# Francis-Fan-create/SCaSML_GP

Measured on AMD Instinct MI355X. Metric: Euler-Maruyama path-steps/sec + L2 rel-error, Grad_Dependent_Nonlinear d=100 n=3, higher is better.
Workload: dtype f32

## Files before the change

scasml_gp_amd/csrc/gp_eval_compat_mfma.hip:

```cpp
#include <stdlib.h>
#include <type_traits>

#include "gp_common.hpp"
#include "gp_mfma16.hpp"

namespace scasml {

constexpr int kHutch = 5;

typedef _Float16 h16x2 __attribute__((ext_vector_type(2)));
typedef float f32x2 __attribute__((ext_vector_type(2)));

struct CompatIdxF {
    int32_t i[kHutch];
};

struct GpCompatArgs {
    const float *points;
    const float *model;
    int32_t idx[kHutch];
    float4 *out4;
    float *lap;
    int64_t n_inf;
    int32_t n_pad, kp, d, first_bdy_tile;
    float a, sigma, mu;
    int32_t eq_id;
    int32_t round_out;
    const uint8_t *site_kinds;
    int64_t rows_per_site;
    const int32_t *site_order;
    int32_t n_listed;
};

template <bool R16>
struct Pair {
    using T = std::conditional_t<R16, h16x2, f32x2>;
    T v;
    __device__ __forceinline__ Pair(float a, float b) {
        if constexpr (R16) v = __builtin_convertvector((f32x2){a, b}, h16x2);
        else v = (f32x2){a, b};
    }
    __device__ __forceinline__ float lo() const { return (float)v.x; }
    __device__ __forceinline__ float hi() const { return (float)v.y; }
};

__device__ __forceinline__ float pin(float x) {
    asm("" : "+v"(x));
    return x;
}

template <int KS, int PLANES>
__device__ __forceinline__ void compat_mfma_lam(const float4 *lds_a, const s16x8 (&xb)[PLANES][KS], f32x16 &acc, int lane, float acc0) {
#pragma unroll
    for (int r = 0; r < 16; ++r) acc[r] = acc0;
    constexpr int NA = PLANES == 2 ? 1 : 2;
    Frag a[NA];
    if constexpr (NA == 2) a[0].f = lds_a[lane];
#pragma unroll
    for (int s = 0; s < KS; ++s) {
        const int cur = NA == 2 ? (s & 1) : 0, nxt = cur ^ 1;
        if constexpr (NA == 2) {
            if (s + 1 < KS) a[nxt].f = lds_a[(s + 1) * 64 + lane];
        } else {
            a[0].f = lds_a[s * 64 + lane];
        }
        Frag b0;
        b0.v = xb[0][s];
        if constexpr (PLANES == 2) {
            Frag b1;
            b1.v = xb[1][s];
            acc = __builtin_amdgcn_mfma_f32_32x32x16_f16(a[cur].h, b1.h, acc, 0, 0, 0);
        }
        acc = __builtin_amdgcn_mfma_f32_32x32x16_f16(a[cur].h, b0.h, acc, 0, 0, 0);
        __builtin_amdgcn_sched_barrier(0);
    }
}

struct CompatPoint {
    float sx, tx, ax0, sx2, wxa, wxb;
};
struct CompatConsts {
    float a, ad, c4, c10;
};

template <int GEOM, int FORM, bool BDY, bool R16>
__device__ __forceinline__ void compat_epilogue(const float *rows_lds, const f32x16 &lam, const f32x16 &G, int half, const CompatPoint &p,
                                                const CompatConsts &c, float &au, float &at, float &ad, float &al) {
    const float4 *cb = reinterpret_cast<const float4 *>(__builtin_assume_aligned(rows_lds + 4 * 8 * half, 16));
    constexpr int NQ = (BDY || GEOM == 1) ? 1 : 2;
    float4 q[1][NQ];
    auto fetch = [&](int r, float4 (&dst)[NQ]) {
        const int row = (r & 3) + 8 * (r >> 2);
#pragma unroll
        for (int i = 0; i < NQ; ++i) dst[i] = cb[row * 2 + i];
    };
#pragma unroll
    for (int r = 0; r < 16; ++r) {
        const int cur = 0;
        fetch(r, q[0]);
        __builtin_amdgcn_sched_barrier(0);
        const float kap = pin(__builtin_amdgcn_exp2f(lam[r]));
        if constexpr (GEOM == 0) {
            const float vsy = q[cur][0].x, vty = q[cur][0].y, c0 = q[cur][0].z;
            if constexpr (BDY && FORM == 1) {
                const Pair<R16> k0(kap, 0.0f);
                au = fmaf(c0, k0.lo(), au);
            } else {
                const float pp = p.tx - vty, ss = p.sx - vsy;
                const float e1 = pin(pp * kap), e2 = pin(ss * kap);
                if constexpr (BDY) {
                    const Pair<R16> k01(kap, e1), k2(e2, 0.0f);
                    au = fmaf(c0, k01.lo(), au);
                    if constexpr (FORM == 0) at = fmaf(-c0, k01.hi(), at);
                    if constexpr (FORM != 1) ad = fmaf(-c0, k2.lo(), ad);
                } else {
                    const float cL = q[cur][0].w, ct = q[cur][1].x, cS = q[cur][1].y;
                    if constexpr (FORM == 1) {
                        const Pair<R16> k01(kap, e1), k2(e2, 0.0f);
                        au = fmaf(cS, k2.lo(), fmaf(ct, k01.hi(), fmaf(c0, k01.lo(), au)));
                    } else {
                        const float e4 = pin(pp * e2);
                        const float e5 = pin(fmaf(-ss, e2, c.ad * kap));
                        if constexpr (FORM == 2) {
                            const Pair<R16> k01(kap, e1), k24(e2, e4), k5(e5, 0.0f);
                            au = fmaf(cS, k24.lo(), fmaf(ct, k01.hi(), fmaf(c0, k01.lo(), au)));
                            ad = fmaf(cS, k5.lo(), fmaf(-ct, k24.hi(), fmaf(-c0, k24.lo(), ad)));
                        } else {
                            const float e3 = fmaf(-pp, e1, c.a * kap);
                            const float g0 = G[r];
                            const float e6 = fmaf(g0, g0 - c.c4, -c.c10) * kap;
                            const Pair<R16> k01(kap, e1), k23(e2, e3), k45(e4, e5), k6(e6, 0.0f);
                            au = fmaf(cS, k23.lo(), fmaf(ct, k01.hi(), fmaf(c0, k01.lo(), au)));
                            at = fmaf(-cS, k45.lo(), fmaf(ct, k23.hi(), fmaf(-c0, k01.hi(), at)));
                            ad = fmaf(cS, k45.hi(), fmaf(-ct, k45.lo(), fmaf(-c0, k23.lo(), ad)));
                            al = fmaf(cL, k6.lo(), al);
                        }
                    }
                }
            }
        } else if constexpr (GEOM == 1) {
            const float vsy1 = q[cur][0].x, vay0 = q[cur][0].y, vwy1 = q[cur][0].z, cL = q[cur][0].w;
            const float g1 = G[r];
            const float f1 = pin(g1 * kap);
            if constexpr (FORM == 1) {
                const Pair<R16> k1(f1, 0.0f);
                au = fmaf(cL, k1.lo(), au);
            } else {
                const float m = fmaf(-(p.sx - vsy1), g1, p.wxb - vwy1);
                const float f3 = pin(m * kap);
                if constexpr (FORM == 2) {
                    const Pair<R16> k13(f1, f3);
                    au = fmaf(cL, k13.lo(), au);
                    ad = fmaf(cL, k13.hi(), ad);
                } else {
                    const float f2 = (p.tx - vay0) * f1;
                    const Pair<R16> k12(f1, f2), k3(f3, 0.0f);
                    au = fmaf(cL, k12.lo(), au);
                    at = fmaf(-cL, k12.hi(), at);
                    ad = fmaf(cL, k3.lo(), ad);
                }
            }
        } else {
            const float vsy = q[cur][0].x, vty = q[cur][0].y, vwy2 = q[cur][0].z, c0 = q[cur][0].w;
            const float g2 = G[r];
            const float h1 = g2 * kap;
            if constexpr (BDY) {
                const Pair<R16> k1(h1, 0.0f);
                al = fmaf(c0, k1.lo(), al);
            } else {
                const float ct = q[cur][1].x, cS = q[cur][1].y;
                const float h2 = (p.ax0 - vty) * h1;
                const float m = fmaf(-(p.sx2 - vsy), g2, p.wxa - vwy2);
                const float h3 = m * kap;
                const Pair<R16> k12(h1, h2), k3(h3, 0.0f);
                al = fmaf(-cS, k3.lo(), fmaf(ct, k12.hi(), fmaf(c0, k12.lo(), al)));
            }
        }
    }
}

template <int GEOM, int FORM, bool BDY>
__device__ __forceinline__ void compat_epilogue_fact(const float *rows_lds, const f32x16 &lam, const f32x16 &G, int half, const CompatPoint &p,
                                                     const CompatConsts &c, float &au, float &at, float &ad, float &al) {
    const float4 *cb = reinterpret_cast<const float4 *>(__builtin_assume_aligned(rows_lds + 4 * 8 * half, 16));
    constexpr int Q0 = GEOM == 2 ? 1 : 0;
    constexpr int NQ = (GEOM == 0 && !BDY) ? 2 : 1;
    float4 q[2][NQ];
    auto fetch = [&](int r, float4 (&dst)[NQ]) {
        const int row = (r & 3) + 8 * (r >> 2);
#pragma unroll
        for (int i = 0; i < NQ; ++i) dst[i] = cb[row * 2 + Q0 + i];
    };
    fetch(0, q[0]);
#pragma unroll
    for (int r = 0; r < 16; ++r) {
        const int cur = r & 1, nxt = cur ^ 1;
        if (r + 1 < 16) fetch(r + 1, q[nxt]);
        #ifndef SCASML_FACT_NOSCHED
        __builtin_amdgcn_sched_barrier(0);
#endif
        const float kap = __builtin_amdgcn_exp2f(lam[r]);
        if constexpr (GEOM == 0) {
            const float vsy = q[cur][0].x, vty = q[cur][0].y, c0 = q[cur][0].z;
            if constexpr (BDY) {
                const float F = c0 * kap;
                au += F;
                if constexpr (FORM == 0) at = fmaf(-(p.tx - vty), F, at);
                if constexpr (FORM != 1) ad = fmaf(-(p.sx - vsy), F, ad);
            } else {
                const float cL = q[cur][0].w, ct = q[cur][1].x, cS = q[cur][1].y;
                const float pp = p.tx - vty, ss = p.sx - vsy;
                const float E = fmaf(ct, pp, fmaf(cS, ss, c0));
                au = fmaf(kap, E, au);
                if constexpr (FORM != 1) ad = fmaf(kap, fmaf(-ss, E, q[cur][1].w), ad);
                if constexpr (FORM == 0) {
                    at = fmaf(kap, fmaf(-pp, E, q[cur][1].z), at);
                    const float g0 = G[r];
                    al = fmaf(cL * kap, fmaf(g0, g0 - c.c4, -c.c10), al);
                }
            }
        } else if constexpr (GEOM == 1) {
            const float vsy1 = q[cur][0].x, vay0 = q[cur][0].y, vwy1 = q[cur][0].z, cL = q[cur][0].w;
            const float v = cL * kap;
            if constexpr (FORM == 1) {
                au = fmaf(v, G[r], au);
            } else {
                const float w = v * G[r];
                au += w;
                ad = fmaf(-(p.sx - vsy1), w, fmaf(v, p.wxb - vwy1, ad));
                if constexpr (FORM == 0) at = fmaf(-(p.tx - vay0), w, at);
            }
        } else {
            const float ct = q[cur][0].x, cS = q[cur][0].y, e0 = q[cur][0].z, cSw = q[cur][0].w;
            if constexpr (BDY) {
                al = fmaf(kap * G[r], e0, al);
            } else {
                const float E2 = fmaf(ct, p.ax0, fmaf(cS, p.sx2, e0));
                const float t = fmaf(cS, p.wxa, -cSw);
                al = fmaf(kap, fmaf(G[r], E2, -t), al);
            }
        }
    }
}

constexpr int kStageTail = 256 + 256;

template <int KS, int BPC, bool R16, int PLANES>
__global__ __launch_bounds__(256, BPC) void gp_eval_compat_mfma_kernel(const GpCompatArgs g) {
    static_assert(PLANES == 2 || !R16, "the as-coded form keeps both point planes");
#ifndef SCASML_COMPAT_NSLOT
#define SCASML_COMPAT_NSLOT 3
#endif
    constexpr int WPB = 4, NSLOT = SCASML_COMPAT_NSLOT, AHEAD = 2;
    constexpr int STAGE = KS * 256 + kStageTail;
    constexpr int NCHUNK = STAGE / 256;
    constexpr int CLO = NCHUNK / WPB, CREM = NCHUNK % WPB;
    extern __shared__ __attribute__((aligned(16))) float lds[];
    const int lane = threadIdx.x & 63, wv = threadIdx.x >> 6;
    const int col = lane & 31, half = lane >> 5;
    const int64_t blk = blockIdx.x;
    int64_t p0 = (blk * WPB + wv) * 32;
    const int n_tiles = g.n_pad / 32;
    const int nb0 = g.first_bdy_tile < n_tiles ? g.first_bdy_tile : n_tiles;

    int form_listed = -1;
    if (g.site_order) {
        const int64_t wps = g.rows_per_site >> 5;
        bool all_u = true, all_ud = true;
        for (int w = 0; w < WPB; ++w) {
            const int64_t vs = (blk * WPB + w) / wps;
            if (vs >= g.n_listed) continue;
            const int k = g.site_kinds ? g.site_kinds[g.site_order[vs]] : 0;
            if (!(k == 1 || k == 3)) all_u = false;
            if (!(k == 1 || k == 3 || k == 4)) all_ud = false;
        }
        form_listed = all_u ? 1 : (all_ud ? 2 : 0);
        const int64_t vw = blk * WPB + wv, vs = vw / wps;
        p0 = vs < g.n_listed ? (int64_t)g.site_order[vs] * g.rows_per_site + (vw - vs * wps) * 32 : g.n_inf;
    }

    if (!g.site_order && g.site_kinds && g.rows_per_site >= 32) {
        const int64_t b0 = blk * WPB * 32;
        if (b0 < g.n_inf) {
            const int64_t b1 = (b0 + WPB * 32 < g.n_inf ? b0 + WPB * 32 : g.n_inf) - 1;
            bool unowned = true;
            for (int64_t s = b0 / g.rows_per_site; s <= b1 / g.rows_per_site; ++s)
                if (g.site_kinds[s] != 2) unowned = false;
            if (unowned) return;
        }
    }
    int form = 0;
    if (g.site_order) {
        form = form_listed;
    } else if (g.site_kinds && g.rows_per_site >= 32) {
        const int64_t b0 = blk * WPB * 32;
        const int64_t b1 = (b0 + WPB * 32 < g.n_inf ? b0 + WPB * 32 : g.n_inf) - 1;
        if (b0 < g.n_inf) {
            bool all_u = true, all_ud = true;
            for (int64_t s = b0 / g.rows_per_site; s <= b1 / g.rows_per_site; ++s) {
                const int k = g.site_kinds[s];
                if (k == 2) continue;
                if (!(k == 1 || k == 3)) all_u = false;
                if (!(k == 1 || k == 3 || k == 4)) all_ud = false;
            }
            form = all_u ? 1 : (all_ud ? 2 : 0);
        }
    }
    form = __builtin_amdgcn_readfirstlane(form);
    const int GD = form == 0 ? 3 : 2, GB = form == 0 ? 2 : 1;
    const int n_stages = nb0 * GD + (n_tiles - nb0) * GB;

    const int wvs = __builtin_amdgcn_readfirstlane(wv);
    const bool extra = wvs < CREM;
    const uint32_t lds_base = __builtin_amdgcn_readfirstlane((uint32_t)(uintptr_t)lds);
    auto stage_src = [&](int s) -> const float * {
        int tile, geom;
        if (s < nb0 * GD) {
            tile = s / GD;
            geom = s - tile * GD;
        } else {
            const int t = s - nb0 * GD;
            tile = nb0 + t / GB;
            geom = form == 0 ? 2 * (t - (t / GB) * GB) : 0;
        }
        return g.model + ((int64_t)tile * 3 + geom) * STAGE;
    };
    auto stage = [&](int s) {
        const uint32_t dst = lds_base + (uint32_t)((s % NSLOT) * STAGE) * 4u;
        const float *src = stage_src(s);
        auto chunk = [&](int c) { glds16_asm(src + c * 256, (uint32_t)lane * 16u, dst + (uint32_t)c * 1024u); };
#pragma unroll
        for (int i = 0; i < CLO; ++i) chunk(wvs + i * WPB);
        if (CREM && extra) chunk(wvs + CLO * WPB);
    };
    auto rendezvous = [&](bool newest_may_fly) {
        if (newest_may_fly) {
            if (CREM && extra) {
                asm volatile("s_waitcnt vmcnt(%0)" ::"n"(CLO + 1) : "memory");
            } else {
                asm volatile("s_waitcnt vmcnt(%0)" ::"n"(CLO) : "memory");
            }
        } else {
            asm volatile("s_waitcnt vmcnt(0)" ::: "memory");
        }
        __builtin_amdgcn_s_barrier();
        asm volatile("" ::: "memory");
    };
    stage(0);
    if (n_stages > 1) stage(1);

    const float qs = 0.5f * 1.44269504088896341f / g.a, k1 = -qs;
    const float hh = (float)g.d / (float)kHutch;
    const float ha2 = hh * g.a * g.a;
    s16x8 xb[PLANES][KS];
    float acc0 = 0.0f;
    CompatPoint pt;
    Frag qa[1], qb[1];
    {
        int64_t row = p0 + col;
        if (row >= g.n_inf) row = g.n_inf - 1;
        const float *prow = g.points + row * g.kp;
        const int kbase = half * (8 * KS);
        const float4 *src = reinterpret_cast<const float4 *>(prow + kbase);
        float pn = 0.0f, ps = 0.0f;
        const float ptime = prow[g.d], px0 = prow[0];
        const float fold = 2.0f * g.a * g.a * qs;
        auto make_planes = [&](const float (&t)[8], Frag &fh, Frag &fl) {
#pragma unroll
            for (int c = 0; c < 4; ++c) {
                const float h0 = (float)(_Float16)t[2 * c], h1 = (float)(_Float16)t[2 * c + 1];
                fh.u[c] = pack_h2(t[2 * c], t[2 * c + 1]);
                fl.u[c] = pack_h2(t[2 * c] - h0, t[2 * c + 1] - h1);
            }
        };
        float tlast[8];
#pragma unroll
        for (int s = 0; s < KS; ++s) {
            const float4 q0 = src[2 * s], q1 = src[2 * s + 1];
            const float e[8] = {q0.x, q0.y, q0.z, q0.w, q1.x, q1.y, q1.z, q1.w};
            float t[8];
#pragma unroll
            for (int c2 = 0; c2 < 8; ++c2) {
                pn = fmaf(e[c2], e[c2], pn);
                ps += e[c2];
                t[c2] = fold * e[c2];
            }
            if (s == KS - 1) {
#pragma unroll
                for (int c2 = 0; c2 < 8; ++c2) tlast[c2] = t[c2];
            } else {
                Frag fh, fl;
                make_planes(t, fh, fl);
                xb[0][s] = fh.v;
                if constexpr (PLANES == 2) xb[1][s] = fl.v;
            }
        }
        pn += __shfl_xor(pn, 32);
        ps += __shfl_xor(ps, 32);
        tlast[5] = half ? 1.0f : tlast[5];
        tlast[6] = half ? 1.0f : tlast[6];
        tlast[7] = half ? k1 * g.a * g.a * pn : tlast[7];
        {
            Frag fh, fl;
            make_planes(tlast, fh, fl);
            xb[0][KS - 1] = fh.v;
            if constexpr (PLANES == 2) xb[1][KS - 1] = fl.v;
            else acc0 = k1 * g.a * g.a * pn - (float)(_Float16)(k1 * g.a * g.a * pn);
        }
        pt.sx = g.a * (ps - ptime);
        pt.tx = g.a * ptime;
        pt.ax0 = g.a * px0;
        pt.sx2 = pt.sx - pt.ax0 + pt.tx;
        float ua[kHutch], ub[kHutch], sa = 0.0f, sb = 0.0f, na = 0.0f, nb = 0.0f;
#pragma unroll
        for (int j = 0; j < kHutch; ++j) {
            const float va = prow[g.idx[j] + 1], vb = prow[g.idx[j]];
            sa += va;
            sb += vb;
            na = fmaf(va, va, na);
            nb = fmaf(vb, vb, nb);
            ua[j] = -2.0f * ha2 * va;
            ub[j] = -2.0f * ha2 * vb;
        }
        pt.wxa = 2.0f * ha2 * sa;
        pt.wxb = 2.0f * ha2 * sb;
        auto qfrag = [&](const float (&u)[kHutch], float px, Frag &f) {
            auto hi = [](float v) { return (float)(_Float16)v; };
            if (half == 0) {
                f.u[0] = pack_h2(u[0], u[1]);
                f.u[1] = pack_h2(u[2], u[3]);
                f.u[2] = pack_h2(u[4], px);
                f.u[3] = pack_h2(px - hi(px), 1.0f);
            } else {
                f.u[0] = pack_h2(u[0] - hi(u[0]), u[1] - hi(u[1]));
                f.u[1] = pack_h2(u[2] - hi(u[2]), u[3] - hi(u[3]));
                f.u[2] = pack_h2(u[4] - hi(u[4]), 1.0f);
                f.u[3] = 0u;
            }
        };
        const float c5ah = (float)kHutch * g.a * hh;
        qfrag(ua, fmaf(ha2, na, -c5ah), qa[0]);
        qfrag(ub, fmaf(ha2, nb, -c5ah), qb[0]);
    }
    CompatConsts cc;
    cc.a = g.a;
    cc.ad = g.a * (float)g.d;
    cc.c4 = 4.0f * g.a * hh;
    cc.c10 = 10.0f * g.a * g.a * hh * hh;
    float au = 0.0f, at = 0.0f, ad = 0.0f, al = 0.0f;
    f32x16 acc, accG;
    uint32_t region;
    asm volatile("s_mov_b32 %0, -1" : "=s"(region));

    int s_now = 0;
    auto step = [&](auto geom_c, auto form_c, auto bdy_c) {
        constexpr int GEOM = decltype(geom_c)::value, FORM = decltype(form_c)::value;
        constexpr bool BDY = decltype(bdy_c)::value;
        constexpr bool NEEDG = GEOM != 0 || (FORM == 0 && !BDY);
        const int slot = s_now % NSLOT;
        if (s_now + AHEAD < n_stages) stage(s_now + AHEAD);
        const float *base = lds + slot * STAGE;
        if (region & 1) {
            compat_mfma_lam<KS, PLANES>(reinterpret_cast<const float4 *>(base), xb, acc, lane, acc0);
            if constexpr (NEEDG) {
                Frag aq;
                aq.f = reinterpret_cast<const float4 *>(base + KS * 256)[lane];
#pragma unroll
                for (int r = 0; r < 16; ++r) accG[r] = 0.0f;
                accG = __builtin_amdgcn_mfma_f32_32x32x16_f16(aq.h, GEOM == 1 ? qb[0].h : qa[0].h, accG, 0, 0, 0);
            }
        }
        if (region & 2) {
            if constexpr (R16) compat_epilogue<GEOM, FORM, BDY, true>(base + (KS + 1) * 256, acc, accG, half, pt, cc, au, at, ad, al);
            else compat_epilogue_fact<GEOM, FORM, BDY>(base + (KS + 1) * 256, acc, accG, half, pt, cc, au, at, ad, al);
        }
        rendezvous(s_now + AHEAD < n_stages);
        ++s_now;
    };
    using I0 = std::integral_constant<int, 0>;
    using I1 = std::integral_constant<int, 1>;
    using I2 = std::integral_constant<int, 2>;
    auto sweep = [&](auto form_c) {
        constexpr int FORM = decltype(form_c)::value;
        for (int jt = 0; jt < nb0; ++jt) {
            step(I0{}, form_c, std::false_type{});
            step(I1{}, form_c, std::false_type{});
            if constexpr (FORM == 0) step(I2{}, form_c, std::false_type{});
        }
        for (int jt = nb0; jt < n_tiles; ++jt) {
            step(I0{}, form_c, std::true_type{});
            if constexpr (FORM == 0) step(I2{}, form_c, std::true_type{});
        }
    };
    rendezvous(n_stages > 1);
    if (form == 2) sweep(I2{});
    else if (form == 1) sweep(I1{});
    else sweep(I0{});

    float u = au + __shfl_xor(au, 32);
    const float dt = at + __shfl_xor(at, 32);
    const float dv = ad + __shfl_xor(ad, 32);
    const float lp = al + __shfl_xor(al, 32);
    const int64_t row = p0 + col;
    if (half == 0 && row < g.n_inf) {
        if (g.round_out) u = (float)(_Float16)u;
        float eps = dt + g.mu * dv + 0.5f * g.sigma * g.sigma * lp + eq_f<float>(g.eq_id, u, g.sigma * dv, g.sigma, (float)g.d);
        if (g.round_out) eps = (float)(_Float16)eps;
        g.out4[row] = make_float4(u, dv, eps, dt);
        if (g.lap) g.lap[row] = lp;
    }
}

__global__ void gp_compat_pack_mfma_kernel(int d, float a, const float *x_dom, int n_dom, const float *x_bdy, int n_bdy, const double *rv,
                                           CompatIdxF ix, float *model, int n_pad, int kp) {
    const int j = blockIdx.x * blockDim.x + threadIdx.x;
    if (j >= n_pad) return;
    const int N = n_dom + n_bdy, D = d + 1, KS = kp / 16;
    const float *src = j < n_dom ? x_dom + (int64_t)j * D : (j < N ? x_bdy + (int64_t)(j - n_dom) * D : nullptr);
    auto y = [&](int k) { return src ? src[k] : 0.0f; };
    const float qs = 0.5f * 1.44269504088896341f / a, k1 = -qs;
    const float hh = (float)d / (float)kHutch, ha2 = hh * a * a;
    float ny = 0.0f, sy = 0.0f;
    for (int k = 0; k < D; ++k) ny = fmaf(y(k), y(k), ny);
    for (int k = 0; k < d; ++k) sy += y(k);
    const float ay = k1 * a * a * ny;
    const _Float16 ayh = (_Float16)ay;
    const float ayl = ay - (float)ayh;
    float c0 = 0.0f, cL = 0.0f, ct = 0.0f, cS = 0.0f;
    if (j < n_dom) {
        c0 = (float)rv[j];
        cL = (float)rv[N + j];
        ct = (float)rv[N + n_dom + j];
        cS = (float)rv[N + 2 * n_dom + j];
    } else if (j < N) {
        c0 = (float)rv[j];
    }
    const int tile = j / 32, i = j % 32;
    const int stage_floats = KS * 256 + kStageTail;
    for (int g = 0; g < 3; ++g) {
        float *blk = model + ((int64_t)tile * 3 + g) * stage_floats;
        uint16_t *planes = reinterpret_cast<uint16_t *>(blk);
        auto yg = [&](int k) { return g == 0 ? y(k) : (g == 1 ? y((k + 1) % D) : y((k + D - 1) % D)); };
        for (int k = 0; k < kp; ++k) {
            const float v = k <= d ? yg(k) : (k == kp - 3 ? (float)ayh : (k == kp - 2 ? ayl : (k == kp - 1 ? 1.0f : 0.0f)));
            const int h = k / (kp / 2), kk = k % (kp / 2);
            const int64_t e = (((int64_t)(kk / 8)) * 64 + h * 32 + i) * 8 + (kk & 7);
            planes[e] = __builtin_bit_cast(unsigned short, (_Float16)v);
        }
        float yq[kHutch], nq = 0.0f, sq = 0.0f;
        for (int q = 0; q < kHutch; ++q) {
            yq[q] = y(ix.i[q] + (g == 2 ? 0 : 1));
            nq = fmaf(yq[q], yq[q], nq);
            sq += yq[q];
        }
        const float py = ha2 * nq;
        const _Float16 pyh = (_Float16)py;
        uint16_t *qf = reinterpret_cast<uint16_t *>(blk + KS * 256);
        auto put = [&](int h, int e, float v) { qf[(h * 32 + i) * 8 + e] = __builtin_bit_cast(unsigned short, (_Float16)v); };
        for (int q = 0; q < kHutch; ++q) {
            put(0, q, yq[q]);
            put(1, q, yq[q]);
        }
        put(0, 5, 1.0f);
        put(0, 6, 1.0f);
        put(0, 7, (float)pyh);
        put(1, 5, py - (float)pyh);
        put(1, 6, 0.0f);
        put(1, 7, 0.0f);
        float *rc = blk + (KS + 1) * 256 + i * 8;
        for (int q = 0; q < 8; ++q) rc[q] = 0.0f;
        if (g == 0) {
            rc[0] = a * sy;
            rc[1] = a * y(d);
            rc[2] = c0;
            rc[3] = cL;
            rc[4] = ct;
            rc[5] = cS;
            rc[6] = a * ct;
            rc[7] = a * (float)d * cS;
        } else if (g == 1) {
            rc[0] = a * (sy - y(0) + y(d));
            rc[1] = a * y(0);
            rc[2] = 2.0f * ha2 * sq;
            rc[3] = cL;
        } else {
            rc[0] = a * sy;
            rc[1] = a * y(d);
            rc[2] = 2.0f * ha2 * sq;
            rc[3] = c0;
            rc[4] = ct;
            rc[5] = cS;
            rc[6] = fmaf(-cS, rc[0], fmaf(-ct, rc[1], c0));
            rc[7] = cS * rc[2];
        }
    }
}

template <int KS, bool R16, int PLANES>
static int launch_compat(const GpCompatArgs &g, hipStream_t s) {
    constexpr int REGS = 4 * PLANES * KS + (R16 ? 72 : 90);
    constexpr size_t lds_bytes = SCASML_COMPAT_NSLOT * (size_t)(KS * 256 + kStageTail) * sizeof(float);
    constexpr int BPC_REGS = REGS <= 128 ? 4 : (REGS <= 164 ? 3 : 2), BPC_LDS = (int)(160 * 1024 / lds_bytes);
    constexpr int BPC = BPC_REGS < BPC_LDS ? BPC_REGS : BPC_LDS;
    const int64_t waves = g.site_order ? (int64_t)g.n_listed * (g.rows_per_site >> 5) : (g.n_inf + 31) / 32;
    const int64_t blocks = (waves + 3) / 4;
    if (blocks == 0) return 0;
    if (blocks > 0x7FFFFFFF) return fail(SCASML_ERR_UNSUPPORTED, "gp_eval_compat_sites: too many points");
    static_assert(lds_bytes * BPC <= 160 * 1024, "LDS slots exceed 160 KiB");
    auto kern = gp_eval_compat_mfma_kernel<KS, BPC, R16, PLANES>;
    if (lds_bytes > 64 * 1024) {
        if (hipFuncSetAttribute(reinterpret_cast<const void *>(kern), hipFuncAttributeMaxDynamicSharedMemorySize, (int)lds_bytes) != hipSuccess)
            return fail(SCASML_ERR_HIP, "gp_eval_compat_sites: cannot reserve %zu bytes of LDS", lds_bytes);
    }
    hipLaunchKernelGGL(kern, dim3((unsigned)blocks), dim3(256), lds_bytes, s, g);
    return check_launch("gp_eval_compat_sites launch");
}

template <bool R16, int PLANES>
static int launch_compat_ks(const GpCompatArgs &g, hipStream_t s) {
    switch (g.kp / 16) {
#define SCASML_CASE(K) \
    case K: return launch_compat<K, R16, PLANES>(g, s);
        SCASML_CASE(1) SCASML_CASE(2) SCASML_CASE(3) SCASML_CASE(4) SCASML_CASE(5) SCASML_CASE(6) SCASML_CASE(7) SCASML_CASE(8)
        SCASML_CASE(9) SCASML_CASE(10) SCASML_CASE(11) SCASML_CASE(12) SCASML_CASE(13) SCASML_CASE(14) SCASML_CASE(15) SCASML_CASE(16)
#undef SCASML_CASE
    }
    return fail(SCASML_ERR_UNSUPPORTED, "gp_eval_compat_sites: kp=%d", g.kp);
}

static int check_idx5(const int32_t *idx_h, int d, int32_t (&out)[kHutch], const char *who) {
    if (!idx_h) return fail(SCASML_ERR_ARG, "%s: idx is null", who);
    for (int j = 0; j < kHutch; ++j) {
        if (idx_h[j] < 0 || idx_h[j] >= d) return fail(SCASML_ERR_ARG, "%s: idx[%d] = %d outside [0, d)", who, j, idx_h[j]);
        for (int q = 0; q < j; ++q)
            if (idx_h[q] == idx_h[j]) return fail(SCASML_ERR_ARG, "%s: idx has a repeated entry %d", who, idx_h[j]);
        out[j] = idx_h[j];
    }
    return 0;
}

}

using namespace scasml;

extern "C" int64_t scasml_gp_compat_model_floats(int32_t d, int32_t n_pad) {
    const int64_t kp = scasml_point_stride(d);
    return (int64_t)(n_pad / SCASML_GP_TILE) * 3 * ((kp / 16) * 256 + kStageTail);
}

extern "C" int scasml_gp_compat_pack_mfma(int32_t d, float a, const float *x_dom, int32_t n_dom, const float *x_bdy, int32_t n_bdy,
                                          const double *rv, const int32_t *idx_h, float *model_out, void *stream) {
    if (!x_dom || !rv || !model_out || (n_bdy > 0 && !x_bdy)) return fail(SCASML_ERR_ARG, "gp_compat_pack_mfma: null argument");
    if (d < kHutch || d > SCASML_MAX_DIM || n_dom < 1 || n_bdy < 0) return fail(SCASML_ERR_ARG, "gp_compat_pack_mfma: bad sizes (d >= %d needed)", kHutch);
    CompatIdxF ix;
    if (int rc = check_idx5(idx_h, d, ix.i, "gp_compat_pack_mfma")) return rc;
    const int n_pad = (n_dom + n_bdy + 31) / 32 * 32;
    const int kp = scasml_point_stride(d);
    hipLaunchKernelGGL(gp_compat_pack_mfma_kernel, dim3((n_pad + 63) / 64), dim3(64), 0, (hipStream_t)stream, d, a, x_dom, n_dom, x_bdy, n_bdy,
                       rv, ix, model_out, n_pad, kp);
    return check_launch("gp_compat_pack_mfma launch");
}

static int eval_compat_sites(int32_t d, float a, float sigma_eq, float mu_eq, int32_t eq_id, const float *model, int32_t n_dom,
                             int32_t n_bdy, const int32_t *idx_h, int32_t round16, float x_bound, const float *points, int64_t n_inf,
                             int64_t rows_per_site, const uint8_t *site_kinds, const int32_t *site_order, int32_t n_listed, float *out4, float *lap,
                             void *stream);

extern "C" int scasml_gp_eval_compat_sites(int32_t d, float a, float sigma_eq, float mu_eq, int32_t eq_id, const float *model, int32_t n_dom,
                                           int32_t n_bdy, const int32_t *idx_h, int32_t round16, float x_bound, const float *points, int64_t n_inf,
                                           int64_t rows_per_site, const uint8_t *site_kinds, float *out4, float *lap, void *stream) {
    return eval_compat_sites(d, a, sigma_eq, mu_eq, eq_id, model, n_dom, n_bdy, idx_h, round16, x_bound, points, n_inf, rows_per_site, site_kinds, nullptr,
                             0, out4, lap, stream);
}

extern "C" int scasml_gp_eval_compat_site_list(int32_t d, float a, float sigma_eq, float mu_eq, int32_t eq_id, const float *model, int32_t n_dom,
                                               int32_t n_bdy, const int32_t *idx_h, int32_t round16, float x_bound, const float *points, int64_t n_inf,
                                               int64_t rows_per_site, const uint8_t *site_kinds, const int32_t *site_order, int32_t n_listed,
                                               float *out4, float *lap, void *stream) {
    if (!site_order || n_listed < 0) return fail(SCASML_ERR_ARG, "gp_eval_compat_site_list: null or negative site list");
    if (rows_per_site < 32 || (rows_per_site & 31)) return fail(SCASML_ERR_ARG, "gp_eval_compat_site_list: rows_per_site must be a positive multiple of 32");
    if (n_inf % rows_per_site) return fail(SCASML_ERR_ARG, "gp_eval_compat_site_list: n_inf must be a whole number of sites");
    if (n_listed > n_inf / rows_per_site) return fail(SCASML_ERR_ARG, "gp_eval_compat_site_list: %d listed sites, the buffer holds %lld", n_listed, (long long)(n_inf / rows_per_site));
    if (n_listed == 0) return 0;
    return eval_compat_sites(d, a, sigma_eq, mu_eq, eq_id, model, n_dom, n_bdy, idx_h, round16, x_bound, points, n_inf, rows_per_site, site_kinds, site_order,
                             n_listed, out4, lap, stream);
}

static int eval_compat_sites(int32_t d, float a, float sigma_eq, float mu_eq, int32_t eq_id, const float *model, int32_t n_dom,
                             int32_t n_bdy, const int32_t *idx_h, int32_t round16, float x_bound, const float *points, int64_t n_inf,
                             int64_t rows_per_site, const uint8_t *site_kinds, const int32_t *site_order, int32_t n_listed, float *out4, float *lap,
                             void *stream) {
    if (n_inf == 0) return 0;
    if (!model || !points || !out4 || n_inf < 0) return fail(SCASML_ERR_ARG, "gp_eval_compat_sites: bad argument");
    if (d < kHutch || d > SCASML_MAX_DIM || n_dom < 1 || n_bdy < 0) return fail(SCASML_ERR_ARG, "gp_eval_compat_sites: bad sizes");
    if (site_kinds && rows_per_site < 1) return fail(SCASML_ERR_ARG, "gp_eval_compat_sites: rows_per_site must be positive");
    if (!eq_known(eq_id)) return fail(SCASML_ERR_UNSUPPORTED, "gp_eval_compat_sites: unknown equation id %d", eq_id);
    const float xb = x_bound > 0.0f ? x_bound : 2.0f;
    if (0.7213f * a * xb * xb * (float)(d + 1) > 3.0e4f)
        return fail(SCASML_ERR_UNSUPPORTED, "gp_eval_compat_sites: a = %g with |x_k| <= %g is outside the fp16 range at d = %d; use scasml_gp_eval_compat",
                    (double)a, (double)xb, d);
    GpCompatArgs g;
    if (int rc = check_idx5(idx_h, d, g.idx, "gp_eval_compat_sites")) return rc;
    g.points = points;
    g.model = model;
    g.out4 = reinterpret_cast<float4 *>(out4);
    g.lap = lap;
    g.n_inf = n_inf;
    g.n_pad = (n_dom + n_bdy + 31) / 32 * 32;
    g.kp = scasml_point_stride(d);
    g.d = d;
    g.first_bdy_tile = (n_dom + SCASML_GP_TILE - 1) / SCASML_GP_TILE;
    g.a = a;
    g.sigma = sigma_eq;
    g.mu = mu_eq;
    g.eq_id = eq_id;
    g.round_out = (round16 & 2) ? 1 : 0;
    g.site_kinds = site_kinds;
    g.rows_per_site = rows_per_site;
    g.site_order = site_order;
    g.n_listed = n_listed;
    hipStream_t s = (hipStream_t)stream;
    if (round16 & 1) {
        if (round16 & 4) return fail(SCASML_ERR_ARG, "gp_eval_compat_sites: round16 bit 2 (one point plane) is the geometry mode's option, not the as-coded form's");
        return launch_compat_ks<true, 2>(g, s);
    }
    return (round16 & 4) ? launch_compat_ks<false, 1>(g, s) : launch_compat_ks<false, 2>(g, s);
}
```

Before: 480.4 million.

## Pack low-plane correction terms into padding to skip last low-plane MFMA

Adds a packed kernel variant used when the K padding has enough slack. The pack kernel places the fp16 low-part corrections of the final input columns, plus the norm and constant terms, into the unused padding slots of the hi plane. This lets the low plane skip its last K-step MFMA in every tile step. It reduces matrix-core work per stage at the cost of extra setup logic and a slightly different rounding arrangement.

```diff
diff --git a/scasml_gp_amd/csrc/gp_eval_compat_mfma.hip b/scasml_gp_amd/csrc/gp_eval_compat_mfma.hip
--- a/scasml_gp_amd/csrc/gp_eval_compat_mfma.hip
+++ b/scasml_gp_amd/csrc/gp_eval_compat_mfma.hip
@@ -32,6 +32,8 @@
     int32_t n_listed;
 };
 
+__host__ __device__ inline bool compat_low_packs(int d, int kp) { return kp >= 32 && kp - d >= 12 && 2 * (d + 1) >= kp; }
+
 template <bool R16>
 struct Pair {
     using T = std::conditional_t<R16, h16x2, f32x2>;
@@ -49,7 +51,7 @@
     return x;
 }
 
-template <int KS, int PLANES>
+template <int KS, int KSL, int PLANES>
 __device__ __forceinline__ void compat_mfma_lam(const float4 *lds_a, const s16x8 (&xb)[PLANES][KS], f32x16 &acc, int lane, float acc0) {
 #pragma unroll
     for (int r = 0; r < 16; ++r) acc[r] = acc0;
@@ -67,9 +69,11 @@
         Frag b0;
         b0.v = xb[0][s];
         if constexpr (PLANES == 2) {
-            Frag b1;
-            b1.v = xb[1][s];
-            acc = __builtin_amdgcn_mfma_f32_32x32x16_f16(a[cur].h, b1.h, acc, 0, 0, 0);
+            if (s < KSL) {
+                Frag b1;
+                b1.v = xb[1][s];
+                acc = __builtin_amdgcn_mfma_f32_32x32x16_f16(a[cur].h, b1.h, acc, 0, 0, 0);
+            }
         }
         acc = __builtin_amdgcn_mfma_f32_32x32x16_f16(a[cur].h, b0.h, acc, 0, 0, 0);
         __builtin_amdgcn_sched_barrier(0);
@@ -247,268 +251,14 @@
 
 template <int KS, int BPC, bool R16, int PLANES>
 __global__ __launch_bounds__(256, BPC) void gp_eval_compat_mfma_kernel(const GpCompatArgs g) {
-    static_assert(PLANES == 2 || !R16, "the as-coded form keeps both point planes");
-#ifndef SCASML_COMPAT_NSLOT
-#define SCASML_COMPAT_NSLOT 3
-#endif
-    constexpr int WPB = 4, NSLOT = SCASML_COMPAT_NSLOT, AHEAD = 2;
-    constexpr int STAGE = KS * 256 + kStageTail;
-    constexpr int NCHUNK = STAGE / 256;
-    constexpr int CLO = NCHUNK / WPB, CREM = NCHUNK % WPB;
-    extern __shared__ __attribute__((aligned(16))) float lds[];
-    const int lane = threadIdx.x & 63, wv = threadIdx.x >> 6;
-    const int col = lane & 31, half = lane >> 5;
-    const int64_t blk = blockIdx.x;
-    int64_t p0 = (blk * WPB + wv) * 32;
-    const int n_tiles = g.n_pad / 32;
-    const int nb0 = g.first_bdy_tile < n_tiles ? g.first_bdy_tile : n_tiles;
-
-    int form_listed = -1;
-    if (g.site_order) {
-        const int64_t wps = g.rows_per_site >> 5;
-        bool all_u = true, all_ud = true;
-        for (int w = 0; w < WPB; ++w) {
-            const int64_t vs = (blk * WPB + w) / wps;
-            if (vs >= g.n_listed) continue;
-            const int k = g.site_kinds ? g.site_kinds[g.site_order[vs]] : 0;
-            if (!(k == 1 || k == 3)) all_u = false;
-            if (!(k == 1 || k == 3 || k == 4)) all_ud = false;
-        }
-        form_listed = all_u ? 1 : (all_ud ? 2 : 0);
-        const int64_t vw = blk * WPB + wv, vs = vw / wps;
-        p0 = vs < g.n_listed ? (int64_t)g.site_order[vs] * g.rows_per_site + (vw - vs * wps) * 32 : g.n_inf;
-    }
-
-    if (!g.site_order && g.site_kinds && g.rows_per_site >= 32) {
-        const int64_t b0 = blk * WPB * 32;
-        if (b0 < g.n_inf) {
-            const int64_t b1 = (b0 + WPB * 32 < g.n_inf ? b0 + WPB * 32 : g.n_inf) - 1;
-            bool unowned = true;
-            for (int64_t s = b0 / g.rows_per_site; s <= b1 / g.rows_per_site; ++s)
-                if (g.site_kinds[s] != 2) unowned = false;
-            if (unowned) return;
-        }
-    }
-    int form = 0;
-    if (g.site_order) {
-        form = form_listed;
-    } else if (g.site_kinds && g.rows_per_site >= 32) {
-        const int64_t b0 = blk * WPB * 32;
-        const int64_t b1 = (b0 + WPB * 32 < g.n_inf ? b0 + WPB * 32 : g.n_inf) - 1;
-        if (b0 < g.n_inf) {
-            bool all_u = true, all_ud = true;
-            for (int64_t s = b0 / g.rows_per_site; s <= b1 / g.rows_per_site; ++s) {
-                const int k = g.site_kinds[s];
-                if (k == 2) continue;
-                if (!(k == 1 || k == 3)) all_u = false;
-                if (!(k == 1 || k == 3 || k == 4)) all_ud = false;
-            }
-            form = all_u ? 1 : (all_ud ? 2 : 0);
-        }
-    }
-    form = __builtin_amdgcn_readfirstlane(form);
-    const int GD = form == 0 ? 3 : 2, GB = form == 0 ? 2 : 1;
-    const int n_stages = nb0 * GD + (n_tiles - nb0) * GB;
-
-    const int wvs = __builtin_amdgcn_readfirstlane(wv);
-    const bool extra = wvs < CREM;
-    const uint32_t lds_base = __builtin_amdgcn_readfirstlane((uint32_t)(uintptr_t)lds);
-    auto stage_src = [&](int s) -> const float * {
-        int tile, geom;
-        if (s < nb0 * GD) {
-            tile = s / GD;
-            geom = s - tile * GD;
-        } else {
-            const int t = s - nb0 * GD;
-            tile = nb0 + t / GB;
-            geom = form == 0 ? 2 * (t - (t / GB) * GB) : 0;
-        }
-        return g.model + ((int64_t)tile * 3 + geom) * STAGE;
-    };
-    auto stage = [&](int s) {
-        const uint32_t dst = lds_base + (uint32_t)((s % NSLOT) * STAGE) * 4u;
-        const float *src = stage_src(s);
-        auto chunk = [&](int c) { glds16_asm(src + c * 256, (uint32_t)lane * 16u, dst + (uint32_t)c * 1024u); };
-#pragma unroll
-        for (int i = 0; i < CLO; ++i) chunk(wvs + i * WPB);
-        if (CREM && extra) chunk(wvs + CLO * WPB);
-    };
-    auto rendezvous = [&](bool newest_may_fly) {
-        if (newest_may_fly) {
-            if (CREM && extra) {
-                asm volatile("s_waitcnt vmcnt(%0)" ::"n"(CLO + 1) : "memory");
-            } else {
-                asm volatile("s_waitcnt vmcnt(%0)" ::"n"(CLO) : "memory");
-            }
-        } else {
-            asm volatile("s_waitcnt vmcnt(0)" ::: "memory");
-        }
-        __builtin_amdgcn_s_barrier();
-        asm volatile("" ::: "memory");
-    };
-    stage(0);
-    if (n_stages > 1) stage(1);
-
-    const float qs = 0.5f * 1.44269504088896341f / g.a, k1 = -qs;
-    const float hh = (float)g.d / (float)kHutch;
-    const float ha2 = hh * g.a * g.a;
-    s16x8 xb[PLANES][KS];
-    float acc0 = 0.0f;
-    CompatPoint pt;
-    Frag qa[1], qb[1];
-    {
-        int64_t row = p0 + col;
-        if (row >= g.n_inf) row = g.n_inf - 1;
-        const float *prow = g.points + row * g.kp;
-        const int kbase = half * (8 * KS);
-        const float4 *src = reinterpret_cast<const float4 *>(prow + kbase);
-        float pn = 0.0f, ps = 0.0f;
-        const float ptime = prow[g.d], px0 = prow[0];
-        const float fold = 2.0f * g.a * g.a * qs;
-        auto make_planes = [&](const float (&t)[8], Frag &fh, Frag &fl) {
-#pragma unroll
-            for (int c = 0; c < 4; ++c) {
-                const float h0 = (float)(_Float16)t[2 * c], h1 = (float)(_Float16)t[2 * c + 1];
-                fh.u[c] = pack_h2(t[2 * c], t[2 * c + 1]);
-                fl.u[c] = pack_h2(t[2 * c] - h0, t[2 * c + 1] - h1);
-            }
-        };
-        float tlast[8];
-#pragma unroll
-        for (int s = 0; s < KS; ++s) {
-            const float4 q0 = src[2 * s], q1 = src[2 * s + 1];
-            const float e[8] = {q0.x, q0.y, q0.z, q0.w, q1.x, q1.y, q1.z, q1.w};
-            float t[8];
-#pragma unroll
-            for (int c2 = 0; c2 < 8; ++c2) {
-                pn = fmaf(e[c2], e[c2], pn);
-                ps += e[c2];
-                t[c2] = fold * e[c2];
-            }
-            if (s == KS - 1) {
-#pragma unroll
-                for (int c2 = 0; c2 < 8; ++c2) tlast[c2] = t[c2];
-            } else {
-                Frag fh, fl;
-                make_planes(t, fh, fl);
-                xb[0][s] = fh.v;
-                if constexpr (PLANES == 2) xb[1][s] = fl.v;
-            }
-        }
-        pn += __shfl_xor(pn, 32);
-        ps += __shfl_xor(ps, 32);
-        tlast[5] = half ? 1.0f : tlast[5];
-        tlast[6] = half ? 1.0f : tlast[6];
-        tlast[7] = half ? k1 * g.a * g.a * pn : tlast[7];
-        {
-            Frag fh, fl;
-            make_planes(tlast, fh, fl);
-            xb[0][KS - 1] = fh.v;
-            if constexpr (PLANES == 2) xb[1][KS - 1] = fl.v;
-            else acc0 = k1 * g.a * g.a * pn - (float)(_Float16)(k1 * g.a * g.a * pn);
-        }
-        pt.sx = g.a * (ps - ptime);
-        pt.tx = g.a * ptime;
-        pt.ax0 = g.a * px0;
-        pt.sx2 = pt.sx - pt.ax0 + pt.tx;
-        float ua[kHutch], ub[kHutch], sa = 0.0f, sb = 0.0f, na = 0.0f, nb = 0.0f;
-#pragma unroll
-        for (int j = 0; j < kHutch; ++j) {
-            const float va = prow[g.idx[j] + 1], vb = prow[g.idx[j]];
-            sa += va;
-            sb += vb;
-            na = fmaf(va, va, na);
-            nb = fmaf(vb, vb, nb);
-            ua[j] = -2.0f * ha2 * va;
-            ub[j] = -2.0f * ha2 * vb;
-        }
-        pt.wxa = 2.0f * ha2 * sa;
-        pt.wxb = 2.0f * ha2 * sb;
-        auto qfrag = [&](const float (&u)[kHutch], float px, Frag &f) {
-            auto hi = [](float v) { return (float)(_Float16)v; };
-            if (half == 0) {
-                f.u[0] = pack_h2(u[0], u[1]);
-                f.u[1] = pack_h2(u[2], u[3]);
-                f.u[2] = pack_h2(u[4], px);
-                f.u[3] = pack_h2(px - hi(px), 1.0f);
-            } else {
-                f.u[0] = pack_h2(u[0] - hi(u[0]), u[1] - hi(u[1]));
-                f.u[1] = pack_h2(u[2] - hi(u[2]), u[3] - hi(u[3]));
-                f.u[2] = pack_h2(u[4] - hi(u[4]), 1.0f);
-                f.u[3] = 0u;
-            }
-        };
-        const float c5ah = (float)kHutch * g.a * hh;
-        qfrag(ua, fmaf(ha2, na, -c5ah), qa[0]);
-        qfrag(ub, fmaf(ha2, nb, -c5ah), qb[0]);
-    }
-    CompatConsts cc;
-    cc.a = g.a;
-    cc.ad = g.a * (float)g.d;
-    cc.c4 = 4.0f * g.a * hh;
-    cc.c10 = 10.0f * g.a * g.a * hh * hh;
-    float au = 0.0f, at = 0.0f, ad = 0.0f, al = 0.0f;
-    f32x16 acc, accG;
-    uint32_t region;
-    asm volatile("s_mov_b32 %0, -1" : "=s"(region));
-
-    int s_now = 0;
-    auto step = [&](auto geom_c, auto form_c, auto bdy_c) {
-        constexpr int GEOM = decltype(geom_c)::value, FORM = decltype(form_c)::value;
-        constexpr bool BDY = decltype(bdy_c)::value;
-        constexpr bool NEEDG = GEOM != 0 || (FORM == 0 && !BDY);
-        const int slot = s_now % NSLOT;
-        if (s_now + AHEAD < n_stages) stage(s_now + AHEAD);
-        const float *base = lds + slot * STAGE;
-        if (region & 1) {
-            compat_mfma_lam<KS, PLANES>(reinterpret_cast<const float4 *>(base), xb, acc, lane, acc0);
-            if constexpr (NEEDG) {
-                Frag aq;
-                aq.f = reinterpret_cast<const float4 *>(base + KS * 256)[lane];
-#pragma unroll
-                for (int r = 0; r < 16; ++r) accG[r] = 0.0f;
-                accG = __builtin_amdgcn_mfma_f32_32x32x16_f16(aq.h, GEOM == 1 ? qb[0].h : qa[0].h, accG, 0, 0, 0);
-            }
-        }
-        if (region & 2) {
-            if constexpr (R16) compat_epilogue<GEOM, FORM, BDY, true>(base + (KS + 1) * 256, acc, accG, half, pt, cc, au, at, ad, al);
-            else compat_epilogue_fact<GEOM, FORM, BDY>(base + (KS + 1) * 256, acc, accG, half, pt, cc, au, at, ad, al);
-        }
-        rendezvous(s_now + AHEAD < n_stages);
-        ++s_now;
-    };
-    using I0 = std::integral_constant<int, 0>;
-    using I1 = std::integral_constant<int, 1>;
-    using I2 = std::integral_constant<int, 2>;
-    auto sweep = [&](auto form_c) {
-        constexpr int FORM = decltype(form_c)::value;
-        for (int jt = 0; jt < nb0; ++jt) {
-            step(I0{}, form_c, std::false_type{});
-            step(I1{}, form_c, std::false_type{});
-            if constexpr (FORM == 0) step(I2{}, form_c, std::false_type{});
-        }
-        for (int jt = nb0; jt < n_tiles; ++jt) {
-            step(I0{}, form_c, std::true_type{});
-            if constexpr (FORM == 0) step(I2{}, form_c, std::true_type{});
-        }
-    };
-    rendezvous(n_stages > 1);
-    if (form == 2) sweep(I2{});
-    else if (form == 1) sweep(I1{});
-    else sweep(I0{});
-
-    float u = au + __shfl_xor(au, 32);
-    const float dt = at + __shfl_xor(at, 32);
-    const float dv = ad + __shfl_xor(ad, 32);
-    const float lp = al + __shfl_xor(al, 32);
-    const int64_t row = p0 + col;
-    if (half == 0 && row < g.n_inf) {
-        if (g.round_out) u = (float)(_Float16)u;
-        float eps = dt + g.mu * dv + 0.5f * g.sigma * g.sigma * lp + eq_f<float>(g.eq_id, u, g.sigma * dv, g.sigma, (float)g.d);
-        if (g.round_out) eps = (float)(_Float16)eps;
-        g.out4[row] = make_float4(u, dv, eps, dt);
-        if (g.lap) g.lap[row] = lp;
-    }
+    constexpr bool PACKED = false;
+#include "gp_eval_compat_mfma_body.hpp"
+}
+
+template <int KS, int BPC, bool R16, int PLANES>
+__global__ __launch_bounds__(256, BPC) void gp_eval_compat_mfma_packed_kernel(const GpCompatArgs g) {
+    constexpr bool PACKED = true;
+#include "gp_eval_compat_mfma_body.hpp"
 }
 
 __global__ void gp_compat_pack_mfma_kernel(int d, float a, const float *x_dom, int n_dom, const float *x_bdy, int n_bdy, const double *rv,
@@ -516,6 +266,7 @@
     const int j = blockIdx.x * blockDim.x + threadIdx.x;
     if (j >= n_pad) return;
     const int N = n_dom + n_bdy, D = d + 1, KS = kp / 16;
+    const bool packs = compat_low_packs(d, kp);
     const float *src = j < n_dom ? x_dom + (int64_t)j * D : (j < N ? x_bdy + (int64_t)(j - n_dom) * D : nullptr);
     auto y = [&](int k) { return src ? src[k] : 0.0f; };
     const float qs = 0.5f * 1.44269504088896341f / a, k1 = -qs;
@@ -542,7 +293,8 @@
         uint16_t *planes = reinterpret_cast<uint16_t *>(blk);
         auto yg = [&](int k) { return g == 0 ? y(k) : (g == 1 ? y((k + 1) % D) : y((k + D - 1) % D)); };
         for (int k = 0; k < kp; ++k) {
-            const float v = k <= d ? yg(k) : (k == kp - 3 ? (float)ayh : (k == kp - 2 ? ayl : (k == kp - 1 ? 1.0f : 0.0f)));
+            float v = k <= d ? yg(k) : (k == kp - 3 ? (float)ayh : (k == kp - 2 ? ayl : (k == kp - 1 ? 1.0f : 0.0f)));
+            if (packs && k > d) v = k == d + 1 ? 1.0f : (k <= d + 9 ? yg(k - (d + 2) + kp / 2 - 8) : (k == kp - 2 ? (float)ayh : (k == kp - 1 ? ayl : 0.0f)));
             const int h = k / (kp / 2), kk = k % (kp / 2);
             const int64_t e = (((int64_t)(kk / 8)) * 64 + h * 32 + i) * 8 + (kk & 7);
             planes[e] = __builtin_bit_cast(unsigned short, (_Float16)v);
@@ -602,12 +354,16 @@
     constexpr size_t lds_bytes = SCASML_COMPAT_NSLOT * (size_t)(KS * 256 + kStageTail) * sizeof(float);
     constexpr int BPC_REGS = REGS <= 128 ? 4 : (REGS <= 164 ? 3 : 2), BPC_LDS = (int)(160 * 1024 / lds_bytes);
     constexpr int BPC = BPC_REGS < BPC_LDS ? BPC_REGS : BPC_LDS;
+    constexpr int REGS_P = REGS + (PLANES == 1 ? 8 : 0);
+    constexpr int BPC_P_REGS = REGS_P <= 128 ? 4 : (REGS_P <= 164 ? 3 : 2), BPC_P = BPC_P_REGS < BPC_LDS ? BPC_P_REGS : BPC_LDS;
     const int64_t waves = g.site_order ? (int64_t)g.n_listed * (g.rows_per_site >> 5) : (g.n_inf + 31) / 32;
     const int64_t blocks = (waves + 3) / 4;
     if (blocks == 0) return 0;
     if (blocks > 0x7FFFFFFF) return fail(SCASML_ERR_UNSUPPORTED, "gp_eval_compat_sites: too many points");
-    static_assert(lds_bytes * BPC <= 160 * 1024, "LDS slots exceed 160 KiB");
+    static_assert(lds_bytes * BPC <= 160 * 1024 && lds_bytes * BPC_P <= 160 * 1024, "LDS slots exceed 160 KiB");
     auto kern = gp_eval_compat_mfma_kernel<KS, BPC, R16, PLANES>;
+    if constexpr (KS >= 2)
+        if (compat_low_packs(g.d, g.kp)) kern = gp_eval_compat_mfma_packed_kernel<KS, BPC_P, R16, PLANES>;
     if (lds_bytes > 64 * 1024) {
         if (hipFuncSetAttribute(reinterpret_cast<const void *>(kern), hipFuncAttributeMaxDynamicSharedMemorySize, (int)lds_bytes) != hipSuccess)
             return fail(SCASML_ERR_HIP, "gp_eval_compat_sites: cannot reserve %zu bytes of LDS", lds_bytes);
diff --git a/scasml_gp_amd/csrc/gp_eval_compat_mfma_body.hpp b/scasml_gp_amd/csrc/gp_eval_compat_mfma_body.hpp
--- /dev/null
+++ b/scasml_gp_amd/csrc/gp_eval_compat_mfma_body.hpp
@@ -0,0 +1,291 @@
+    static_assert(PLANES == 2 || !R16, "the as-coded form keeps both point planes");
+    static_assert(!PACKED || KS >= 2, "the packed layout needs two K-steps");
+#ifndef SCASML_COMPAT_NSLOT
+#define SCASML_COMPAT_NSLOT 3
+#endif
+    constexpr int WPB = 4, NSLOT = SCASML_COMPAT_NSLOT, AHEAD = 2;
+    constexpr int STAGE = KS * 256 + kStageTail;
+    constexpr int NCHUNK = STAGE / 256;
+    constexpr int CLO = NCHUNK / WPB, CREM = NCHUNK % WPB;
+    extern __shared__ __attribute__((aligned(16))) float lds[];
+    const int lane = threadIdx.x & 63, wv = threadIdx.x >> 6;
+    const int col = lane & 31, half = lane >> 5;
+    const int64_t blk = blockIdx.x;
+    int64_t p0 = (blk * WPB + wv) * 32;
+    const int n_tiles = g.n_pad / 32;
+    const int nb0 = g.first_bdy_tile < n_tiles ? g.first_bdy_tile : n_tiles;
+
+    int form_listed = -1;
+    if (g.site_order) {
+        const int64_t wps = g.rows_per_site >> 5;
+        bool all_u = true, all_ud = true;
+        for (int w = 0; w < WPB; ++w) {
+            const int64_t vs = (blk * WPB + w) / wps;
+            if (vs >= g.n_listed) continue;
+            const int k = g.site_kinds ? g.site_kinds[g.site_order[vs]] : 0;
+            if (!(k == 1 || k == 3)) all_u = false;
+            if (!(k == 1 || k == 3 || k == 4)) all_ud = false;
+        }
+        form_listed = all_u ? 1 : (all_ud ? 2 : 0);
+        const int64_t vw = blk * WPB + wv, vs = vw / wps;
+        p0 = vs < g.n_listed ? (int64_t)g.site_order[vs] * g.rows_per_site + (vw - vs * wps) * 32 : g.n_inf;
+    }
+
+    if (!g.site_order && g.site_kinds && g.rows_per_site >= 32) {
+        const int64_t b0 = blk * WPB * 32;
+        if (b0 < g.n_inf) {
+            const int64_t b1 = (b0 + WPB * 32 < g.n_inf ? b0 + WPB * 32 : g.n_inf) - 1;
+            bool unowned = true;
+            for (int64_t s = b0 / g.rows_per_site; s <= b1 / g.rows_per_site; ++s)
+                if (g.site_kinds[s] != 2) unowned = false;
+            if (unowned) return;
+        }
+    }
+    int form = 0;
+    if (g.site_order) {
+        form = form_listed;
+    } else if (g.site_kinds && g.rows_per_site >= 32) {
+        const int64_t b0 = blk * WPB * 32;
+        const int64_t b1 = (b0 + WPB * 32 < g.n_inf ? b0 + WPB * 32 : g.n_inf) - 1;
+        if (b0 < g.n_inf) {
+            bool all_u = true, all_ud = true;
+            for (int64_t s = b0 / g.rows_per_site; s <= b1 / g.rows_per_site; ++s) {
+                const int k = g.site_kinds[s];
+                if (k == 2) continue;
+                if (!(k == 1 || k == 3)) all_u = false;
+                if (!(k == 1 || k == 3 || k == 4)) all_ud = false;
+            }
+            form = all_u ? 1 : (all_ud ? 2 : 0);
+        }
+    }
+    form = __builtin_amdgcn_readfirstlane(form);
+    const int GD = form == 0 ? 3 : 2, GB = form == 0 ? 2 : 1;
+    const int n_stages = nb0 * GD + (n_tiles - nb0) * GB;
+
+    const int wvs = __builtin_amdgcn_readfirstlane(wv);
+    const bool extra = wvs < CREM;
+    const uint32_t lds_base = __builtin_amdgcn_readfirstlane((uint32_t)(uintptr_t)lds);
+    auto stage_src = [&](int s) -> const float * {
+        int tile, geom;
+        if (s < nb0 * GD) {
+            tile = s / GD;
+            geom = s - tile * GD;
+        } else {
+            const int t = s - nb0 * GD;
+            tile = nb0 + t / GB;
+            geom = form == 0 ? 2 * (t - (t / GB) * GB) : 0;
+        }
+        return g.model + ((int64_t)tile * 3 + geom) * STAGE;
+    };
+    auto stage = [&](int s) {
+        const uint32_t dst = lds_base + (uint32_t)((s % NSLOT) * STAGE) * 4u;
+        const float *src = stage_src(s);
+        auto chunk = [&](int c) { glds16_asm(src + c * 256, (uint32_t)lane * 16u, dst + (uint32_t)c * 1024u); };
+#pragma unroll
+        for (int i = 0; i < CLO; ++i) chunk(wvs + i * WPB);
+        if (CREM && extra) chunk(wvs + CLO * WPB);
+    };
+    auto rendezvous = [&](bool newest_may_fly) {
+        if (newest_may_fly) {
+            if (CREM && extra) {
+                asm volatile("s_waitcnt vmcnt(%0)" ::"n"(CLO + 1) : "memory");
+            } else {
+                asm volatile("s_waitcnt vmcnt(%0)" ::"n"(CLO) : "memory");
+            }
+        } else {
+            asm volatile("s_waitcnt vmcnt(0)" ::: "memory");
+        }
+        __builtin_amdgcn_s_barrier();
+        asm volatile("" ::: "memory");
+    };
+    stage(0);
+    if (n_stages > 1) stage(1);
+
+    const float qs = 0.5f * 1.44269504088896341f / g.a, k1 = -qs;
+    const float hh = (float)g.d / (float)kHutch;
+    const float ha2 = hh * g.a * g.a;
+    s16x8 xb[PLANES][KS];
+    float acc0 = 0.0f;
+    CompatPoint pt;
+    Frag qa[1], qb[1];
+    {
+        int64_t row = p0 + col;
+        if (row >= g.n_inf) row = g.n_inf - 1;
+        const float *prow = g.points + row * g.kp;
+        const int kbase = half * (8 * KS);
+        const float4 *src = reinterpret_cast<const float4 *>(prow + kbase);
+        float pn = 0.0f, ps = 0.0f;
+        const float ptime = prow[g.d], px0 = prow[0];
+        const float fold = 2.0f * g.a * g.a * qs;
+        auto make_planes = [&](const float (&t)[8], Frag &fh, Frag &fl) {
+#pragma unroll
+            for (int c = 0; c < 4; ++c) {
+                const float h0 = (float)(_Float16)t[2 * c], h1 = (float)(_Float16)t[2 * c + 1];
+                fh.u[c] = pack_h2(t[2 * c], t[2 * c + 1]);
+                fl.u[c] = pack_h2(t[2 * c] - h0, t[2 * c + 1] - h1);
+            }
+        };
+        constexpr int NL = PACKED ? (KS < 3 ? KS : 3) : 1;
+        float tlast[NL][8];
+#pragma unroll
+        for (int s = 0; s < KS; ++s) {
+            const float4 q0 = src[2 * s], q1 = src[2 * s + 1];
+            const float e[8] = {q0.x, q0.y, q0.z, q0.w, q1.x, q1.y, q1.z, q1.w};
+            float t[8];
+#pragma unroll
+            for (int c2 = 0; c2 < 8; ++c2) {
+                pn = fmaf(e[c2], e[c2], pn);
+                ps += e[c2];
+                t[c2] = fold * e[c2];
+            }
+            if (s >= KS - NL) {
+#pragma unroll
+                for (int c2 = 0; c2 < 8; ++c2) tlast[s - (KS - NL)][c2] = t[c2];
+            } else {
+                Frag fh, fl;
+                make_planes(t, fh, fl);
+                xb[0][s] = fh.v;
+                if constexpr (PLANES == 2) xb[1][s] = fl.v;
+            }
+        }
+        pn += __shfl_xor(pn, 32);
+        ps += __shfl_xor(ps, 32);
+        if constexpr (!PACKED) {
+            tlast[0][5] = half ? 1.0f : tlast[0][5];
+            tlast[0][6] = half ? 1.0f : tlast[0][6];
+            tlast[0][7] = half ? k1 * g.a * g.a * pn : tlast[0][7];
+            Frag fh, fl;
+            make_planes(tlast[0], fh, fl);
+            xb[0][KS - 1] = fh.v;
+            if constexpr (PLANES == 2) xb[1][KS - 1] = fl.v;
+            else acc0 = k1 * g.a * g.a * pn - (float)(_Float16)(k1 * g.a * g.a * pn);
+        } else {
+            const float n2 = k1 * g.a * g.a * pn;
+            const int off = g.kp - g.d - 10;
+#pragma unroll
+            for (int j = 0; j < NL; ++j) {
+                const int s = KS - NL + j;
+#pragma unroll
+                for (int c2 = 0; c2 < 8; ++c2) {
+                    const int k = half * (g.kp >> 1) + 8 * s + c2, m = k - (g.d + 2);
+                    float vl = 0.0f;
+                    if constexpr (PLANES == 2) {
+                        const float v = fold * prow[8 * s + c2 + off];
+                        vl = (float)(_Float16)(v - (float)(_Float16)v);
+                    }
+                    if (k == g.d + 1) tlast[j][c2] = n2;
+                    else if (m >= 0 && m < 8) tlast[j][c2] = vl;
+                    else if (k >= g.kp - 2) tlast[j][c2] = 1.0f;
+                }
+                Frag fh, fl;
+                make_planes(tlast[j], fh, fl);
+                xb[0][s] = fh.v;
+                if constexpr (PLANES == 2) xb[1][s] = fl.v;
+            }
+            if constexpr (PLANES == 1) acc0 = n2 - (float)(_Float16)n2;
+        }
+        pt.sx = g.a * (ps - ptime);
+        pt.tx = g.a * ptime;
+        pt.ax0 = g.a * px0;
+        pt.sx2 = pt.sx - pt.ax0 + pt.tx;
+        float ua[kHutch], ub[kHutch], sa = 0.0f, sb = 0.0f, na = 0.0f, nb = 0.0f;
+#pragma unroll
+        for (int j = 0; j < kHutch; ++j) {
+            const float va = prow[g.idx[j] + 1], vb = prow[g.idx[j]];
+            sa += va;
+            sb += vb;
+            na = fmaf(va, va, na);
+            nb = fmaf(vb, vb, nb);
+            ua[j] = -2.0f * ha2 * va;
+            ub[j] = -2.0f * ha2 * vb;
+        }
+        pt.wxa = 2.0f * ha2 * sa;
+        pt.wxb = 2.0f * ha2 * sb;
+        auto qfrag = [&](const float (&u)[kHutch], float px, Frag &f) {
+            auto hi = [](float v) { return (float)(_Float16)v; };
+            if (half == 0) {
+                f.u[0] = pack_h2(u[0], u[1]);
+                f.u[1] = pack_h2(u[2], u[3]);
+                f.u[2] = pack_h2(u[4], px);
+                f.u[3] = pack_h2(px - hi(px), 1.0f);
+            } else {
+                f.u[0] = pack_h2(u[0] - hi(u[0]), u[1] - hi(u[1]));
+                f.u[1] = pack_h2(u[2] - hi(u[2]), u[3] - hi(u[3]));
+                f.u[2] = pack_h2(u[4] - hi(u[4]), 1.0f);
+                f.u[3] = 0u;
+            }
+        };
+        const float c5ah = (float)kHutch * g.a * hh;
+        qfrag(ua, fmaf(ha2, na, -c5ah), qa[0]);
+        qfrag(ub, fmaf(ha2, nb, -c5ah), qb[0]);
+    }
+    CompatConsts cc;
+    cc.a = g.a;
+    cc.ad = g.a * (float)g.d;
+    cc.c4 = 4.0f * g.a * hh;
+    cc.c10 = 10.0f * g.a * g.a * hh * hh;
+    constexpr int KSL = PACKED && PLANES == 2 ? KS - 1 : KS;
+    float au = 0.0f, at = 0.0f, ad = 0.0f, al = 0.0f;
+    f32x16 acc, accG;
+    uint32_t region;
+    asm volatile("s_mov_b32 %0, -1" : "=s"(region));
+
+    int s_now = 0;
+    auto step = [&](auto geom_c, auto form_c, auto bdy_c) {
+        constexpr int GEOM = decltype(geom_c)::value, FORM = decltype(form_c)::value;
+        constexpr bool BDY = decltype(bdy_c)::value;
+        constexpr bool NEEDG = GEOM != 0 || (FORM == 0 && !BDY);
+        const int slot = s_now % NSLOT;
+        if (s_now + AHEAD < n_stages) stage(s_now + AHEAD);
+        const float *base = lds + slot * STAGE;
+        if (region & 1) {
+            compat_mfma_lam<KS, KSL, PLANES>(reinterpret_cast<const float4 *>(base), xb, acc, lane, acc0);
+            if constexpr (NEEDG) {
+                Frag aq;
+                aq.f = reinterpret_cast<const float4 *>(base + KS * 256)[lane];
+#pragma unroll
+                for (int r = 0; r < 16; ++r) accG[r] = 0.0f;
+                accG = __builtin_amdgcn_mfma_f32_32x32x16_f16(aq.h, GEOM == 1 ? qb[0].h : qa[0].h, accG, 0, 0, 0);
+            }
+        }
+        if (region & 2) {
+            if constexpr (R16) compat_epilogue<GEOM, FORM, BDY, true>(base + (KS + 1) * 256, acc, accG, half, pt, cc, au, at, ad, al);
+            else compat_epilogue_fact<GEOM, FORM, BDY>(base + (KS + 1) * 256, acc, accG, half, pt, cc, au, at, ad, al);
+        }
+        rendezvous(s_now + AHEAD < n_stages);
+        ++s_now;
+    };
+    using I0 = std::integral_constant<int, 0>;
+    using I1 = std::integral_constant<int, 1>;
+    using I2 = std::integral_constant<int, 2>;
+    auto sweep = [&](auto form_c) {
+        constexpr int FORM = decltype(form_c)::value;
+        for (int jt = 0; jt < nb0; ++jt) {
+            step(I0{}, form_c, std::false_type{});
+            step(I1{}, form_c, std::false_type{});
+            if constexpr (FORM == 0) step(I2{}, form_c, std::false_type{});
+        }
+        for (int jt = nb0; jt < n_tiles; ++jt) {
+            step(I0{}, form_c, std::true_type{});
+            if constexpr (FORM == 0) step(I2{}, form_c, std::true_type{});
+        }
+    };
+    rendezvous(n_stages > 1);
+    if (form == 2) sweep(I2{});
+    else if (form == 1) sweep(I1{});
+    else sweep(I0{});
+
+    float u = au + __shfl_xor(au, 32);
+    const float dt = at + __shfl_xor(at, 32);
+    const float dv = ad + __shfl_xor(ad, 32);
+    const float lp = al + __shfl_xor(al, 32);
+    int col_end = col;
+    if constexpr (PACKED) asm("" : "+v"(col_end));
+    const int64_t row = p0 + col_end;
+    if (half == 0 && row < g.n_inf) {
+        if (g.round_out) u = (float)(_Float16)u;
+        float eps = dt + g.mu * dv + 0.5f * g.sigma * g.sigma * lp + eq_f<float>(g.eq_id, u, g.sigma * dv, g.sigma, (float)g.d);
+        if (g.round_out) eps = (float)(_Float16)eps;
+        g.out4[row] = make_float4(u, dv, eps, dt);
+        if (g.lap) g.lap[row] = lp;
+    }
```

Result: faster. 486.1 million (median of 6 runs) (+1.2%).
